# carlosmwh1985/BspAtom

Hardware: AMD Instinct MI355X
Metric: l-channel eigensolves/sec at N_bsp=4096 fp64 (higher is better)
Workload: dtype f64; 1 GPU; Hydrogen Coulomb l=0..127, N_bsp=4096, k=9, KIND_GRID=0 rb=800 (BASELINE configs[3]); `value` = weak scaling: 128 l-channels per GPU, 128 in total; channels_total=128, eigenvector_owner_rank=0, collective_calls=0, launched_by=python

## Files before the change

### bspatom_amd/csrc/capi.hip

```cpp
#include <atomic>
#include <new>
#include "capi_internal.h"

using namespace bsp;

namespace bsp {
static std::atomic<int> g_process_device{-1};
int process_device() { return g_process_device.load(); }
int process_device_check(int device)
{
    const int cur = g_process_device.load();
    if (cur >= 0 && cur != device) {
        fprintf(stderr, "bspatom: this process already works on device %d; use one process per GPU (device %d refused)\n", cur, device);
        return BSP_ERR_UNSUPPORTED;
    }
    return BSP_OK;
}
void process_device_latch(int device) { int expect = -1; g_process_device.compare_exchange_strong(expect, device); }
}

namespace {
struct OptName { const char *name; const char *env; int Options::*field; };
const OptName OPT_TABLE[] = {
    {"sb2st_version", "BSP_SB2ST_VERSION", &Options::sb2st_version},
    {"sb2st_ring", "BSP_SB2ST_RING", &Options::sb2st_ring},
    {"sb2st_margin", "BSP_SB2ST_MARGIN", &Options::sb2st_margin},
    {"sb2st_hyst", "BSP_SB2ST_HYST", &Options::sb2st_hyst},
    {"sb2st_lead", "BSP_SB2ST_LEAD", &Options::sb2st_lead},
    {"sb2st_check", "BSP_SB2ST_CHECK", &Options::sb2st_check},
    {"sb2st_diag", "BSP_SB2ST_DIAG", &Options::sb2st_diag},
    {"sb2st_force_abort", "BSP_SB2ST_FORCE_ABORT", &Options::sb2st_force_abort},
    {"sy2sb_groups", "BSP_SY2SB_GROUPS", &Options::sy2sb_groups},
    {"sy2sb_lookahead", "BSP_SY2SB_LOOKAHEAD", &Options::sy2sb_lookahead},
    {"sy2sb_segs", "BSP_SY2SB_SEGS", &Options::sy2sb_segs},
    {"panel_qr", "BSP_PANEL_QR", &Options::panel_qr},
    {"gemm_diag", "BSP_GEMM_DIAG", &Options::gemm_diag},
    {"bisect", "BSP_BISECT", &Options::bisect},
    {"bisect_ept", "BSP_BISECT_EPT", &Options::bisect_ept},
    {"bisect_tail", "BSP_BISECT_TAIL", &Options::bisect_tail},
    {"bisect_secant", "BSP_BISECT_SECANT", &Options::bisect_secant},
    {"bisect_pair", "BSP_BISECT_PAIR", &Options::bisect_pair},
    {"bisect_diag", "BSP_BISECT_DIAG", &Options::bisect_diag},
    {"no_eigvec_prefetch", "BSP_NO_EIGVEC_PREFETCH", &Options::no_eigvec_prefetch},
    {"vec_early", "BSP_VEC_EARLY", &Options::vec_early},
    {"vec_own_cu", "BSP_VEC_OWN_CU", &Options::vec_own_cu},
    {"poison_c", "BSP_POISON_C", &Options::poison_c},
    {"sb2sb_mfma", "BSP_SB2SB_MFMA", &Options::sb2sb_mfma},
    {"ktime", "BSP_KTIME", &Options::ktime},
    {"tsqr_regcap", "BSP_TSQR_REGCAP", &Options::tsqr_regcap},
    {"tsqr_max_m", "BSP_TSQR_MAX_M", &Options::tsqr_max_m},
    {"sb16_rows", "BSP_SB16_ROWS", &Options::sb16_rows},
    {"route", "BSP_ROUTE", &Options::route},
    {"cw_onediv", "BSP_CW_ONEDIV", &Options::cw_onediv},
    {"cw_items4", "BSP_CW_ITEMS4", &Options::cw_items4},
    {"cw_nw", "BSP_CW_NW", &Options::cw_nw},
    {"cw_ldspad", "BSP_CW_LDSPAD", &Options::cw_ldspad},
    {"cw_ipw", "BSP_CW_IPW", &Options::cw_ipw},
    {"cw_band8", "BSP_CW_BAND8", &Options::cw_band8},
    {"cw_split", "BSP_CW_SPLIT", &Options::cw_split},
    {"cw_diag", "BSP_CW_DIAG", &Options::cw_diag},
    {"s_overlap", "BSP_S_OVERLAP", &Options::s_overlap},
    {"cw_streams", "BSP_CW_STREAMS", &Options::cw_streams},
    {"cw_chunk_min", "BSP_CW_CHUNK_MIN", &Options::cw_chunk_min},
    {"sb8_wgs", "BSP_SB8_WGS", &Options::sb8_wgs},
    {"sbr_phased", "BSP_SBR_PHASED", &Options::sbr_phased},
    {"sbr_lag", "BSP_SBR_LAG", &Options::sbr_lag},
    {"fused_probe", "BSP_FUSED_PROBE", &Options::fused_probe},
    {"dipole_stage_mb", "BSP_DIPOLE_STAGE_MB", &Options::dipole_stage_mb},
    {"wf_stage_mb", "BSP_WF_STAGE_MB", &Options::wf_stage_mb},
    {"tdse_stage_mb", "BSP_TDSE_STAGE_MB", &Options::tdse_stage_mb},
};
}

namespace bsp {
Options &opts()
{
    static Options o = [] {
        Options v;
        for (const OptName &t : OPT_TABLE) {
            const char *e = getenv(t.env);
            if (e) v.*(t.field) = (*e == 0) ? 1 : atoi(e);
        }
        return v;
    }();
    return o;
}

namespace {
struct KRec { int slot; hipEvent_t e0, e1; };
std::vector<KRec> g_krecs;
std::vector<hipEvent_t> g_kpool;
hipEvent_t g_kopen[KS_COUNT];
hipEvent_t kevent()
{
    hipEvent_t e = nullptr;
    if (!g_kpool.empty()) { e = g_kpool.back(); g_kpool.pop_back(); }
    else if (hipEventCreate(&e) != hipSuccess) e = nullptr;
    return e;
}
const char *const KSLOT_NAMES[KS_COUNT] = {"gemm2_kernel<128,128,MODE 1> (rank-128 update, syr2k)", "gemm2_kernel<64,128,MODE 2> (symm Y = A22 W)",
                                          "panel_qr2_kernel / panel_qr_kernel", "sy2sb chain: G, K (split-K gemm_kernel + splitk_reduce), form_T, tsmm64 (W, Z)",
                                          "sb2sb_mfma_kernel (band 64 -> 16)", "sbr_rows_kernel<8> / <16> / sb16st_kernel (one-column chase to tridiagonal)", "bisect3_kernel",
                                          "band_cholesky_kernel + std_form_kernel",
                                          "crawford_item_kernel and its set-up kernels (band route: pencil -> band 15)",
                                          "operator_band_kernel (bands of caller-given g(r), g(r) d/dr)",
                                          "tdse_stage_kernel (one Runge-Kutta stage of bspatom_tdse_propagate)"};
}
void ktime_begin(int slot, hipStream_t st)
{
    hipEvent_t e = kevent();
    g_kopen[slot] = e;
    if (e) (void)hipEventRecord(e, st);
}
void ktime_end(int slot, hipStream_t st)
{
    hipEvent_t e0 = g_kopen[slot], e1 = kevent();
    g_kopen[slot] = nullptr;
    if (!e0 || !e1) return;
    (void)hipEventRecord(e1, st);
    g_krecs.push_back({slot, e0, e1});
}
}

extern "C" int bspatom_kernel_times(double *ms, int32_t *launches, int cap)
// ... 481 lines not shown
```

### bspatom_amd/csrc/common.h

```cpp
#pragma once
#include <hip/hip_runtime.h>
#include <cstdint>
#include <cstdio>
#include <cstdlib>

#define BSP_OK 0
#define BSP_ERR_HIP (-1)
#define BSP_ERR_ARG (-2)
#define BSP_ERR_BSPLVB (-3)
#define BSP_ERR_NOGPU (-4)
#define BSP_ERR_UNSUPPORTED (-5)

#define BSP_HIP(x)                                                                          \
    do {                                                                                    \
        hipError_t e_ = (x);                                                                \
        if (e_ != hipSuccess) {                                                             \
            fprintf(stderr, "bspatom: HIP error '%s' at %s:%d\n", hipGetErrorString(e_),    \
                    __FILE__, __LINE__);                                                    \
            return BSP_ERR_HIP;                                                             \
        }                                                                                   \
    } while (0)

typedef double double4_t __attribute__((ext_vector_type(4)));

__host__ __device__ inline size_t ab_stride(int npad) { return (size_t)npad * 128 + 1088; }

namespace bsp {

struct Options {
    int sb2st_version = 0;
    int sb2st_ring = 0;
    int sb2st_margin = 3, sb2st_hyst = 2;
    int sb2st_lead = 0;
    int sb2st_check = 0;
    int sb2st_diag = 0;
    int sb2st_force_abort = 0;
    int sy2sb_groups = 2, sy2sb_lookahead = 1, sy2sb_segs = 0;
    int panel_qr = 3;
    int tsqr_max_m = 2048;
    int tsqr_regcap = 1;
    int gemm_diag = 0;
    int bisect = 3, bisect_ept = 0;
    int bisect_secant = 1;
    int bisect_tail = 1;
    int bisect_pair = 1;
    int bisect_diag = 0;
    int no_eigvec_prefetch = 0;
    int vec_early = 1;
    int vec_own_cu = 1;
    int sb2sb_mfma = 1;
    int sb16_rows = 1;
    int poison_c = 0;
    int route = 0;
    int fused_probe = 0;
    int cw_items4 = 1;
    int cw_nw = 1;
    int cw_streams = 2;
    int cw_chunk_min = 1024;
    int s_overlap = 1;
    int cw_diag = 0;
    int cw_split = 0;
    int cw_band8 = 1;
    int sb8_wgs = 0;
    int sbr_phased = 1;
    int sbr_lag = 0;
    int cw_ipw = 0;
    int cw_ldspad = 0;
    int cw_onediv = 0;
    int dipole_stage_mb = 0;
    int wf_stage_mb = 0;
    int tdse_stage_mb = 0;
    int ktime = 0;
};
Options &opts();

int process_device();
int process_device_check(int device);
void process_device_latch(int device);

enum KSlot { KS_SYR2K = 0, KS_SYMM, KS_PANEL_QR, KS_CHAIN, KS_SB2SB, KS_SB16ST, KS_BISECT, KS_STDFORM, KS_CRAWFORD, KS_OPBAND, KS_TDSE, KS_COUNT };
void ktime_begin(int slot, hipStream_t st);
void ktime_end(int slot, hipStream_t st);
struct KScope {
    int slot; hipStream_t st; bool on;
    KScope(int slot_, hipStream_t st_) : slot(slot_), st(st_), on(opts().ktime != 0) { if (on) ktime_begin(slot, st); }
    ~KScope() { if (on) ktime_end(slot, st); }
};

struct GemmDesc {
    int M, N, K, batch;
    const double *A; long sAm, sAk, bA;
    const double *B; long sBk, sBn, bB;
    double *C; long sCm, sCn, bC;
    double alpha, beta;
    int lower_only;
    int yoff;
    int ksplit;
    int kchunk;
    long bCs;
    int nsb, toff;
    int sbpre[80];
    int sbxy[80];
};
int gemm_f64(const GemmDesc &g, hipStream_t st);
int gemm_splitk_f64(const GemmDesc &g, int splits, double *part, hipStream_t st);
int tsmm64_f64(int m, int batch, const double *A, long lda, long bsA, const double *B, long bsB, double *C, long ldc, long bsC,
               double alpha, double beta, hipStream_t st);
int syr2k_lower_f64(int m, int batch, double *A22, long ld, long bsA, const double *buf, long ldb, long bsBuf, int seg, int nseg,
                    int part, hipStream_t st);
int symm_lower_f64(int m, int batch, const double *A22, long ld, long bsA, const double *W, long ldw, long bsW,
                   double *Y, long ldy, long bsY, hipStream_t st);

int launch_point_table(int nkp, int k, int ka, int nfun, const double *d_rt, const double *d_aind,
                       const double *d_xg, const double *d_wg, const double *d_vpot, double *d_ptab,
                       int *d_left, int *d_status, hipStream_t st);
int launch_assemble_bands(int nfun, int k, int ka, int nkp, int kind_pot, const double *d_bl, int l0,
                          int nl, const double *d_ptab, const int *d_left, double *d_SB, double *d_HB,
                          hipStream_t st);
int launch_dipole_bands(int nfun, int k, int ka, int nkp, const double *d_ptab, const int *d_left, double *d_RB,
                        hipStream_t st);
int launch_band_cholesky(int n, int k, const double *d_SB, double *d_UB, double *d_rdiag, int *d_info,
                         hipStream_t st);
int launch_band_cholesky_range(int n, int k, int jstart, int jstop, const double *d_SB, double *d_UB, double *d_rdiag, int *d_info,
                               hipStream_t st);
int launch_band_cholesky_pair(int n, int k, int jstop, const double *d_SB, double *d_UB, double *d_rdiag, int *d_info, hipStream_t st);
int launch_standard_form(int n, int npad, int k, int nl, const double *d_HB, const double *d_UB,
                         const double *d_rdiag, double *d_Y, double *d_C, hipStream_t st, int full = 0);
struct CrawfordWork {
// ... 109 lines not shown
```

### bspatom_amd/csrc/tridiag.hip

```cpp
#include <vector>
#include "common.h"

namespace bsp {

__device__ __forceinline__ int sturm_count(const double *__restrict__ d, const double *__restrict__ e2,
                                           int n, double x, double pivmin)
{
    double q = d[0] - x;
    if (fabs(q) < pivmin) q = -pivmin;
    int cnt = (q < 0.0) ? 1 : 0;
    for (int i = 1; i < n; ++i) {
        q = (d[i] - x) - e2[i - 1] / q;
        if (fabs(q) < pivmin) q = -pivmin;
        cnt += (q < 0.0) ? 1 : 0;
    }
    return cnt;
}

constexpr int EPT = 4;

__global__ __launch_bounds__(256) void bisect_kernel(int n, int ldn, const double *__restrict__ dall,
                                                    const double *__restrict__ eall, double *wall, long ldw)
{
    extern __shared__ double sm[];
    double *d = sm, *e2 = sm + n;
    __shared__ double red[8];
    const int tid = threadIdx.x;
    const size_t ch = blockIdx.y;
    const double *dg = dall + ch * (size_t)ldn, *eg = eall + ch * (size_t)ldn;
    double gl = 1e300, gu = -1e300, emax = 0.0;
    for (int i = tid; i < n; i += 256) {
        const double di = dg[i];
        const double el = (i > 0) ? fabs(eg[i - 1]) : 0.0;
        const double er = (i < n - 1) ? fabs(eg[i]) : 0.0;
        d[i] = di;
        e2[i] = (i < n - 1) ? eg[i] * eg[i] : 0.0;
        gl = fmin(gl, di - el - er);
        gu = fmax(gu, di + el + er);
        emax = fmax(emax, er * er);
    }
#pragma unroll
    for (int off = 32; off >= 1; off >>= 1) {
        gl = fmin(gl, __shfl_xor(gl, off));
        gu = fmax(gu, __shfl_xor(gu, off));
        emax = fmax(emax, __shfl_xor(emax, off));
    }
    if ((tid & 63) == 0) { red[tid >> 6] = gl; red[4 + (tid >> 6)] = gu; }
    __syncthreads();
    gl = fmin(fmin(red[0], red[1]), fmin(red[2], red[3]));
    gu = fmax(fmax(red[4], red[5]), fmax(red[6], red[7]));
    __syncthreads();
    if ((tid & 63) == 0) red[tid >> 6] = emax;
    __syncthreads();
    emax = fmax(fmax(red[0], red[1]), fmax(red[2], red[3]));
    const double safmin = 2.2250738585072014e-308;
    const double pivmin = safmin * fmax(1.0, emax);
    const double tnorm = fmax(fabs(gl), fabs(gu));
    const double eps = 2.220446049250313e-16;
    gl = gl - 2.1 * tnorm * eps * n - 2.1 * pivmin;
    gu = gu + 2.1 * tnorm * eps * n + 2.1 * pivmin;

    const int mbase = blockIdx.x * (256 * EPT) + tid;
    double lo[EPT], hi[EPT];
#pragma unroll
    for (int c = 0; c < EPT; ++c) { lo[c] = gl; hi[c] = gu; }
    for (int it = 0; it < 128; ++it) {
        double mid[EPT];
        bool done[EPT];
        bool alld = true;
#pragma unroll
        for (int c = 0; c < EPT; ++c) {
            mid[c] = 0.5 * (lo[c] + hi[c]);
            done[c] = (mid[c] <= lo[c]) || (mid[c] >= hi[c]) ||
                      (hi[c] - lo[c] <= 2.0 * eps * fmax(fabs(lo[c]), fabs(hi[c])) + 2.0 * pivmin);
            alld = alld && done[c];
        }
        if (__syncthreads_and(alld)) break;
        double q[EPT];
        int cnt[EPT];
        {
            const double d0 = d[0];
#pragma unroll
// ... 137 lines not shown
            _Pragma("unroll") for (int r = 0; r < RS; ++r) {                                          \
                const double2 v = LOADROW(ib + sb * RS + r + 1);                                      \
                _Pragma("unroll") for (int c = 0; c < EPT; ++c) {                                     \
                    const double pn = __builtin_fma(v.x - x[c], p1[c], -(v.y * p0[c]));               \
                    h[c] = __builtin_amdgcn_alignbit(h[c], (unsigned)__double2hiint(pn), 31);         \
                    p0[c] = p1[c];                                                                    \
                    p1[c] = pn;                                                                       \
                }                                                                                     \
            }                                                                                         \
            _Pragma("unroll") for (int c = 0; c < EPT; ++c) {                                         \
                const int ex = -__builtin_amdgcn_frexp_exp(p1[c]);      \
                p1[c] = __builtin_amdgcn_ldexp(p1[c], ex);                                            \
                p0[c] = __builtin_amdgcn_ldexp(p0[c], ex);                                            \
                if (VAL) es[c] -= ex;                                            \
            }                                                                                         \
        }                                                                                             \
        _Pragma("unroll") for (int c = 0; c < EPT; ++c) {                                             \
            const unsigned t = __builtin_amdgcn_alignbit(hp[c], h[c], 1);                             \
            cnt[c] += __builtin_popcount(h[c] ^ t);                                                   \
            hp[c] = h[c];                                                                             \
        }                                                                                             \
    }
__device__ __forceinline__ double2 sturm_gload(const double2 *p)
{
    typedef double d2v __attribute__((ext_vector_type(2)));
    const d2v v = __builtin_nontemporal_load(reinterpret_cast<const d2v *>(p));
    return make_double2(v.x, v.y);
}
template <int EPT, bool VAL = false>
__device__ __forceinline__ void sturm_counts3(const double2 *__restrict__ de, int np, const double (&x)[EPT], int (&cnt)[EPT],
                                              const double2 *__restrict__ gt = nullptr, int nl = 0x7fffffff, float *lf = nullptr)
{
    double p0[EPT], p1[EPT];
    unsigned h[EPT], hp[EPT];
    int es[EPT];
#pragma unroll
    for (int c = 0; c < EPT; ++c) es[c] = 0;
    const double d0 = de[0].x;
#pragma unroll
    for (int c = 0; c < EPT; ++c) {
        p0[c] = 1.0; p1[c] = d0 - x[c];
        hp[c] = (unsigned)__double2hiint(p1[c]) >> 31;
        cnt[c] = (int)hp[c]; h[c] = 0u;
    }
    const int nlds = nl < np ? nl : np;
#define STURM_LDS(i) de[i]
#define STURM_GLB(i) sturm_gload(gt + (i))
    for (int ib = 0; ib < nlds; ib += HW) STURM_BLOCK(STURM_LDS)
    for (int ib = nlds; ib < np; ib += HW) STURM_BLOCK(STURM_GLB)
#undef STURM_LDS
#undef STURM_GLB
    if (VAL) {
#pragma unroll
        for (int c = 0; c < EPT; ++c) {
            const int e2 = __builtin_amdgcn_frexp_exp(p1[c]);
            const float mant = (float)__builtin_amdgcn_ldexp(p1[c], -e2);
            lf[c] = (float)(es[c] + e2) + __log2f(fmaxf(fabsf(mant), 1e-30f));
        }
    }
}

__device__ __forceinline__ double msect_point(double a, double w, int q, double rp)
{
    return __builtin_fma(w, (double)(q + 1) * rp, a);
}

__device__ __forceinline__ bool bracket_final(double lo, double hi)
{
    const double mid = 0.5 * (lo + hi);
    return (mid <= lo) || (mid >= hi) || (hi - lo <= 2.0 * 2.220446049250313e-16 * fmax(fabs(lo), fabs(hi)) + 1e-300);
}

__device__ __forceinline__ double uniform_double(double v)
{
    return __hiloint2double(__builtin_amdgcn_readfirstlane(__double2hiint(v)), __builtin_amdgcn_readfirstlane(__double2loint(v)));
}

static size_t bisect3_lds_bytes(int n, int ng)
{
    const int np = (n + HW - 1) / HW * HW;
    return (size_t)(np + 1) * 16 + (size_t)(ng / 2) * 16 + (size_t)ng * 4 + (size_t)(ng / 2) * 4;
}

constexpr int BISECT_DIAG_WORDS = 8;
template <int EPT, int TPB, bool DIAG = false>
__global__ __launch_bounds__(TPB) void bisect3_kernel(int n, int ldn, const double *__restrict__ dall,
                                                     const double *__restrict__ eall, double *wall, long ldw, int tail,
                                                     double2 *gtail, int nl, int hybrid_arg, int pair_stride, long long *diag)
{
    long long dt0 = DIAG ? (long long)wall_clock64() : 0;
    const int hybrid = EPT > 4 ? 0 : hybrid_arg;
    extern __shared__ double2 sde[];
    constexpr int NG = TPB * EPT;
    constexpr int NW = TPB / 64;
    constexpr int KC = NG / 2;
    const int np = (n + HW - 1) / HW * HW;
    const int nlr = nl < np ? nl : np;
    double2 *de = sde;
    const int kcap = hybrid ? NG / 4 : KC;
    double *llo = (double *)(sde + nlr + 1);
    double *lhi = llo + kcap;
    int *cg = (int *)(lhi + kcap);
    int *lm = cg + NG;
    __shared__ double red[2 * NW];
    __shared__ int sK;
    const int tid0 = threadIdx.x;
    const size_t ch = blockIdx.y;
    const double *dg = dall + ch * (size_t)ldn, *eg = eall + ch * (size_t)ldn;
    double *wout = wall + ch * (size_t)ldw;
    double2 *gt = gtail ? gtail + ch * (size_t)(np + 1) : nullptr;
    double gl = 1e300, gu = -1e300;
    for (int i = tid0; i < n; i += TPB) {
        const double di = dg[i];
        const double el = (i > 0) ? fabs(eg[i - 1]) : 0.0;
        const double er = (i < n - 1) ? fabs(eg[i]) : 0.0;
        gl = fmin(gl, di - el - er);
        gu = fmax(gu, di + el + er);
    }
#pragma unroll
    for (int off = 32; off >= 1; off >>= 1) {
        gl = fmin(gl, __shfl_xor(gl, off));
        gu = fmax(gu, __shfl_xor(gu, off));
    }
    if ((tid0 & 63) == 0) { red[tid0 >> 6] = gl; red[NW + (tid0 >> 6)] = gu; }
    __syncthreads();
#pragma unroll
    for (int q = 0; q < NW; ++q) { gl = fmin(gl, red[q]); gu = fmax(gu, red[NW + q]); }
    const double eps = 2.220446049250313e-16;
    double tnorm = fmax(fabs(gl), fabs(gu));
    if (!(tnorm > 0.0)) tnorm = 1.0;
    int kexp;
    (void)frexp(tnorm, &kexp);
    const double sc = ldexp(1.0, -kexp), isc_v = ldexp(1.0, kexp);
    for (int i = tid0; i <= np; i += TPB) {
        const double di = (i < n) ? dg[i] * sc : 2.0;
        const double ev = (i >= 1 && i < n) ? (eg[i - 1] * sc) : 0.0;
        const double2 row = make_double2(di, fmax(ev * ev, 1e-60));
        if (i <= nlr) de[i] = row; else gt[i] = row;
    }
    if (gt) asm volatile("s_waitcnt vmcnt(0)" ::: "memory");
    __syncthreads();
    gl = gl * sc - 2.1 * eps * n - 1e-300;
    gu = gu * sc + 2.1 * eps * n + 1e-300;

    gl = uniform_double(gl); gu = uniform_double(gu);
    const double isc = uniform_double(isc_v);
    const int nwl = (n + NG - 1) / NG;
#pragma unroll 1
    for (int item = 0; item < 2; ++item) {
        const int bx = blockIdx.x + item * pair_stride;
        if (item) {
            if (pair_stride == 0 || bx >= nwl) break;
            __syncthreads();
            if (DIAG) dt0 = (long long)wall_clock64();
        }
        int drounds = 0, dtail = 0;
        int tid = tid0;
        asm volatile("" : "+v"(tid));
        const int mbase = bx * NG + tid;
        double lo[EPT], hi[EPT];
        int clo[EPT], chi[EPT];
        float lflo[EPT], lfhi[EPT];
        if (!hybrid) {
            const double w = gu - gl;
            double xg[EPT];
            int cc[EPT];
#pragma unroll
            for (int c = 0; c < EPT; ++c) xg[c] = gl + w * ((double)(tid + TPB * c + 1) * (1.0 / (NG + 1)));
            if (DIAG) ++drounds;
            sturm_counts3<EPT>(de, np, xg, cc, gt, nlr);
#pragma unroll
            for (int c = 0; c < EPT; ++c) cg[tid + TPB * c] = cc[c];
            __syncthreads();
#pragma unroll
            for (int c = 0; c < EPT; ++c) {
                const int m = mbase + TPB * c;
                int L = -1, R = NG;
                while (R - L > 1) {
                    const int mid = (L + R) >> 1;
                    if (cg[mid] > m) R = mid; else L = mid;
                }
                lo[c] = (L < 0) ? gl : gl + w * ((double)(L + 1) * (1.0 / (NG + 1)));
                hi[c] = (R >= NG) ? gu : gl + w * ((double)(R + 1) * (1.0 / (NG + 1)));
                clo[c] = (L < 0) ? 0 : cg[L];
                chi[c] = (R >= NG) ? n : cg[R];
            }
        }
        bool done[EPT];
        if (hybrid) {
            double *xs = llo;
            float *lfs = (float *)(xs + NG);
            unsigned short *cs = (unsigned short *)(lfs + NG);
            const int m0 = bx * NG, m1 = min(m0 + NG, n);
            float wref[EPT];
            int st[EPT];
#pragma unroll
            for (int c = 0; c < EPT; ++c) {
                wref[c] = 3e38f; st[c] = 0;
                lo[c] = gl; hi[c] = gu; clo[c] = 0; chi[c] = n; lflo[c] = 3e38f; lfhi[c] = 3e38f;
            }
            for (int it = 0; it < 200; ++it) {
                double x[EPT];
                bool sec[EPT];
                int rng[EPT];
#pragma unroll
                for (int c = 0; c < EPT; ++c) {
                    const int m = mbase + TPB * c;
                    const double wd = hi[c] - lo[c];
                    done[c] = (m >= n) || bracket_final(lo[c], hi[c]);
                    if ((float)wd <= 0.5f * wref[c]) { wref[c] = (float)wd; st[c] &= 3; }
                    const bool slow = (st[c] >> 2) >= 3;
                    st[c] += 4;
                    x[c] = 0.5 * (lo[c] + hi[c]); sec[c] = false; rng[c] = 0;
                    const int a = max(clo[c], m0), b = min(chi[c], m1);
                    if (chi[c] - clo[c] == 1 && lflo[c] < 1e38f && lfhi[c] < 1e38f && !slow && !done[c]) {
                        const double tiny = 2.0 * 2.220446049250313e-16 * fmax(fabs(lo[c]), fabs(hi[c]));
                        const float dl = fminf(fmaxf(lflo[c] - lfhi[c], -60.0f), 60.0f);
                        const double r = (double)exp2f(dl);
                        const double xe = fmin(fmax(lo[c] + wd * (r / (1.0 + r)), lo[c] + tiny), hi[c] - tiny);
                        if (xe > lo[c] && xe < hi[c]) { x[c] = xe; sec[c] = true; }
                    } else if (b - a > 1 && m >= a && m < b && !slow && !done[c]) {
                        const double xq = msect_point(lo[c], wd, m - a, 1.0 / (double)(b - a + 1));
                        if (xq > lo[c] && xq < hi[c]) { x[c] = xq; rng[c] = (a - m0) | ((b - m0) << 16); }
                    }
                }
                int tot = 0;
#pragma unroll
                for (int c = 0; c < EPT; ++c) tot += __syncthreads_count(!done[c]);
                if (tot <= (tail ? NG / hybrid : 0)) break;
                int cnt[EPT];
                float lf[EPT];
                if (DIAG) ++drounds;
                sturm_counts3<EPT, true>(de, np, x, cnt, gt, nlr, lf);
#pragma unroll
                for (int c = 0; c < EPT; ++c) {
                    xs[tid + TPB * c] = x[c]; cs[tid + TPB * c] = (unsigned short)cnt[c]; lfs[tid + TPB * c] = lf[c];
                }
// ... 43 lines not shown
            for (int c = 0; c < EPT; ++c) {
                if (!done[c]) {
                    if (cnt[c] > mbase + TPB * c) hi[c] = mid[c]; else lo[c] = mid[c];
                }
            }
        }
        if (tid == 0) sK = 0;
        __syncthreads();
#pragma unroll
        for (int c = 0; c < EPT; ++c) {
            const int m = mbase + TPB * c;
            done[c] = (m >= n) || bracket_final(lo[c], hi[c]);
            if (!done[c]) {
                const int pos = atomicAdd(&sK, 1);
                if (pos < kcap) { llo[pos] = lo[c]; lhi[pos] = hi[c]; lm[pos] = m; }
                else wout[m] = 0.5 * (lo[c] + hi[c]) * isc;
            } else if (m < n) wout[m] = 0.5 * (lo[c] + hi[c]) * isc;
        }
        __syncthreads();
        for (int round = 0; round < 128; ++round) {
            const int K = min(sK, kcap);
            if (K == 0) break;
            const int P = NG / K;
            const double rp = 1.0 / (double)(P + 1);
            double x[EPT];
            int cc[EPT];
#pragma unroll
            for (int c = 0; c < EPT; ++c) {
                const int s = tid + TPB * c, e = s / P, q = s - e * P;
                x[c] = 2.0;
                if (e < K) { const double a = llo[e]; x[c] = msect_point(a, lhi[e] - a, q, rp); }
            }
            if (DIAG) ++dtail;
            sturm_counts3<EPT>(de, np, x, cc, gt, nlr);
#pragma unroll
            for (int c = 0; c < EPT; ++c) cg[tid + TPB * c] = cc[c];
            __syncthreads();
            double nlo[EPT / 2], nhi[EPT / 2];
            int nm[EPT / 2];
            bool keep[EPT / 2];
#pragma unroll
            for (int j = 0; j < EPT / 2; ++j) {
                const int e = tid + TPB * j;
                keep[j] = false;
                if (e < K) {
                    const double a = llo[e], b = lhi[e], w = b - a;
                    const int m = lm[e];
                    const int *ce = cg + e * P;
                    int L = -1, R = P;
                    while (R - L > 1) {
                        const int mid = (L + R) >> 1;
                        if (ce[mid] > m) R = mid; else L = mid;
                    }
                    nlo[j] = (L < 0) ? a : msect_point(a, w, L, rp);
                    nhi[j] = (R >= P) ? b : msect_point(a, w, R, rp);
                    nm[j] = m;
                    if (bracket_final(nlo[j], nhi[j]) || !(nhi[j] - nlo[j] < w)) wout[m] = 0.5 * (nlo[j] + nhi[j]) * isc;
                    else keep[j] = true;
                }
            }
            __syncthreads();
            if (tid == 0) sK = 0;
            __syncthreads();
#pragma unroll
            for (int j = 0; j < EPT / 2; ++j) {
                if (keep[j]) {
                    const int pos = atomicAdd(&sK, 1);
                    llo[pos] = nlo[j]; lhi[pos] = nhi[j]; lm[pos] = nm[j];
                }
            }
            __syncthreads();
        }
        {
            const int K = min(sK, kcap);
            for (int e = tid; e < K; e += TPB) wout[lm[e]] = 0.5 * (llo[e] + lhi[e]) * isc;
        }
        if (DIAG && tid == 0) {
            long long *rec = diag + (ch * (size_t)nwl + bx) * BISECT_DIAG_WORDS;
            rec[0] = bx; rec[1] = (long long)ch;
            rec[2] = (long long)(__builtin_amdgcn_s_getreg((31 << 11) | 20) & 0xfu);
            rec[3] = (long long)(unsigned)__builtin_amdgcn_s_getreg((31 << 11) | 4);
            rec[4] = dt0; rec[5] = (long long)wall_clock64();
            rec[6] = drounds; rec[7] = dtail;
        }
    }
}

__global__ __launch_bounds__(64) void bisect_one_kernel(int n, const double *__restrict__ dg, const double *__restrict__ eg,
                                                       int m, double *out)
{
    extern __shared__ double sm[];
    const int np = (n + RS - 1) / RS * RS;
    double *d = sm, *e2 = sm + np + RS;
    const int lane = threadIdx.x;
    double gl = 1e300, gu = -1e300;
    for (int i = lane; i < n; i += 64) {
        const double di = dg[i];
        const double el = (i > 0) ? fabs(eg[i - 1]) : 0.0;
        const double er = (i < n - 1) ? fabs(eg[i]) : 0.0;
        gl = fmin(gl, di - el - er);
        gu = fmax(gu, di + el + er);
    }
#pragma unroll
    for (int off = 32; off >= 1; off >>= 1) {
        gl = fmin(gl, __shfl_xor(gl, off));
        gu = fmax(gu, __shfl_xor(gu, off));
    }
    const double eps = 2.220446049250313e-16;
    double tnorm = fmax(fabs(gl), fabs(gu));
    if (!(tnorm > 0.0)) tnorm = 1.0;
    int kexp;
    (void)frexp(tnorm, &kexp);
    const double sc = ldexp(1.0, -kexp), isc = ldexp(1.0, kexp);
    for (int i = lane; i < np + RS; i += 64) {
        d[i] = (i < n) ? dg[i] * sc : 2.0;
        const double ev = (i < n - 1) ? (eg[i] * sc) : 0.0;
        e2[i] = fmax(ev * ev, 1e-60);
    }
    __syncthreads();
    double lo = gl * sc - 2.1 * eps * n - 1e-300, hi = gu * sc + 2.1 * eps * n + 1e-300;
    for (int round = 0; round < 40; ++round) {
        if (hi - lo <= 2.0 * eps * fmax(fabs(lo), fabs(hi)) + 1e-300) break;
        const double w = (hi - lo) * (1.0 / 65.0);
        const double x = lo + (lane + 1) * w;
        if (!(x > lo && x < hi)) {
            const double mid = 0.5 * (lo + hi);
            if (!(mid > lo && mid < hi)) break;
        }
        double p0 = 1.0, p1 = d[0] - x;
        int cnt = (p1 < 0.0) ? 1 : 0;
        for (int ib = 0; ib < np; ib += RS) {
#pragma unroll
            for (int r = 0; r < RS; ++r) {
                const int i = ib + r + 1;
                const double pn = __builtin_fma(d[i] - x, p1, -(e2[i - 1] * p0));
                cnt += (int)((unsigned)(__double2hiint(pn) ^ __double2hiint(p1)) >> 31);
                p0 = p1; p1 = pn;
            }
            int ea, eb;
            (void)frexp(p1, &ea);
            (void)frexp(p0, &eb);
            const int ex = (p1 == 0.0) ? eb : ((p0 == 0.0) ? ea : max(ea, eb));
            p1 = ldexp(p1, -ex); p0 = ldexp(p0, -ex);
        }
        const unsigned long long above = __ballot(cnt > m);
        const int f = above ? (__ffsll((long long)above) - 1) : 64;
        const double xl = __shfl(x, f > 0 ? f - 1 : 0), xh = __shfl(x, f < 64 ? f : 63);
        const double nlo = (f > 0) ? xl : lo, nhi = (f < 64) ? xh : hi;
        if (!(nhi - nlo < hi - lo)) break;
        lo = nlo; hi = nhi;
    }
    if (lane == 0) *out = 0.5 * (lo + hi) * isc;
}

__global__ __launch_bounds__(256) void bisect_one3_kernel(int n, const double *__restrict__ dg, const double *__restrict__ eg,
                                                         int m, double *out)
{
    extern __shared__ double2 sde[];
    constexpr int NG = 256 * EPT;
    const int np = (n + HW - 1) / HW * HW;
    double2 *de = sde;
    int *cg = (int *)(sde + np + 1);
    __shared__ double red[8];
    const int tid = threadIdx.x;
    double gl = 1e300, gu = -1e300;
    for (int i = tid; i < n; i += 256) {
// ... 48 lines not shown
        lo = nlo; hi = nhi;
    }
    if (tid == 0) *out = 0.5 * (lo + hi) * isc;
}

int launch_bisect_one(int n, const double *d_d, const double *d_e, int m, double *d_out, hipStream_t st)
{
    const int variant1 = opts().bisect;
    if (variant1 >= 3) {
        const size_t lds3 = (size_t)2 * (n + 3 * RS + HW) * sizeof(double) + 256 * EPT * sizeof(int);
        if (lds3 > 150 * 1024) return BSP_ERR_UNSUPPORTED;
        static bool attr3 = false;
        if (!attr3) {
            BSP_HIP(hipFuncSetAttribute(reinterpret_cast<const void *>(bisect_one3_kernel),
                                        hipFuncAttributeMaxDynamicSharedMemorySize, 150 * 1024));
            attr3 = true;
        }
        hipLaunchKernelGGL(bisect_one3_kernel, dim3(1), dim3(256), lds3, st, n, d_d, d_e, m, d_out);
        BSP_HIP(hipGetLastError());
        return BSP_OK;
    }
    const size_t lds = (size_t)2 * (n + 3 * RS) * sizeof(double);
    if (lds > 150 * 1024) return BSP_ERR_UNSUPPORTED;
    static bool attr = false;
    if (!attr) {
        BSP_HIP(hipFuncSetAttribute(reinterpret_cast<const void *>(bisect_one_kernel),
                                    hipFuncAttributeMaxDynamicSharedMemorySize, 150 * 1024));
        attr = true;
    }
    hipLaunchKernelGGL(bisect_one_kernel, dim3(1), dim3(64), lds, st, n, d_d, d_e, m, d_out);
    BSP_HIP(hipGetLastError());
    return BSP_OK;
}

int launch_bisect(int n, int ldn, int batch, const double *d_d, const double *d_e, double *d_w, long ldw,
                  hipStream_t st)
{
    const int ept_env = opts().bisect_ept;
    int mode = (ept_env == 8) ? 8 : (ept_env == 4) ? 4 : (ept_env == 2) ? 1024 : (ept_env == 21) ? 21 : (ept_env == 5) ? 512 : 22;
    int ng = (mode == 4) ? 1024 : (mode == 21 ? 512 : (mode == 22 ? 1024 : 2048));
    if (bisect3_lds_bytes(n, ng) > 150 * 1024) { mode = 22; ng = 1024; }
    const int np3 = (n + HW - 1) / HW * HW;
    int nl = np3;
    while (bisect3_lds_bytes(nl, ng) > 150 * 1024) nl -= HW;
    const size_t lds3 = bisect3_lds_bytes(nl, ng);
    const size_t lds = (size_t)2 * (n + 3 * RS + HW) * sizeof(double);
    struct Tail { hipStream_t st; double2 *p; size_t cap; };
    static std::vector<Tail> g_tails;
    double2 *gtail = nullptr;
    if (nl < np3) {
        const size_t need = (size_t)batch * (np3 + 1);
        Tail *tl = nullptr;
        for (auto &x : g_tails) if (x.st == st) tl = &x;
        if (!tl) { g_tails.push_back({st, nullptr, 0}); tl = &g_tails.back(); }
        if (need > tl->cap) {
            if (tl->p) { BSP_HIP(hipStreamSynchronize(st)); (void)hipFree(tl->p); tl->p = nullptr; tl->cap = 0; }
            BSP_HIP(hipMalloc(reinterpret_cast<void **>(&tl->p), need * sizeof(double2)));
            tl->cap = need;
        }
        gtail = tl->p;
        if (opts().bisect < 3) return BSP_ERR_UNSUPPORTED;
    }
    static bool attr_set = false;
    const int variant = opts().bisect;
    if (!attr_set) {
        BSP_HIP(hipFuncSetAttribute(reinterpret_cast<const void *>(bisect_kernel),
                                    hipFuncAttributeMaxDynamicSharedMemorySize, 150 * 1024));
        BSP_HIP(hipFuncSetAttribute(reinterpret_cast<const void *>(bisect2_kernel),
                                    hipFuncAttributeMaxDynamicSharedMemorySize, 150 * 1024));
        BSP_HIP(hipFuncSetAttribute(reinterpret_cast<const void *>(bisect3_kernel<4, 256>),
                                    hipFuncAttributeMaxDynamicSharedMemorySize, 150 * 1024));
        BSP_HIP(hipFuncSetAttribute(reinterpret_cast<const void *>(bisect3_kernel<8, 256>),
                                    hipFuncAttributeMaxDynamicSharedMemorySize, 150 * 1024));
        BSP_HIP(hipFuncSetAttribute(reinterpret_cast<const void *>(bisect3_kernel<4, 512>),
                                    hipFuncAttributeMaxDynamicSharedMemorySize, 150 * 1024));
        BSP_HIP(hipFuncSetAttribute(reinterpret_cast<const void *>(bisect3_kernel<2, 1024>),
                                    hipFuncAttributeMaxDynamicSharedMemorySize, 150 * 1024));
        BSP_HIP(hipFuncSetAttribute(reinterpret_cast<const void *>(bisect3_kernel<2, 256>),
                                    hipFuncAttributeMaxDynamicSharedMemorySize, 150 * 1024));
        BSP_HIP(hipFuncSetAttribute(reinterpret_cast<const void *>(bisect3_kernel<2, 512>),
                                    hipFuncAttributeMaxDynamicSharedMemorySize, 150 * 1024));
        BSP_HIP(hipFuncSetAttribute(reinterpret_cast<const void *>(bisect3_kernel<2, 512, true>),
                                    hipFuncAttributeMaxDynamicSharedMemorySize, 150 * 1024));
        attr_set = true;
    }
    const dim3 grid((n + 256 * EPT - 1) / (256 * EPT), batch);
    if (variant == 1 || variant == 2) {
        KScope kt(KS_BISECT, st);
        if (variant == 1) hipLaunchKernelGGL(bisect_kernel, grid, dim3(256), lds, st, n, ldn, d_d, d_e, d_w, ldw);
        else hipLaunchKernelGGL(bisect2_kernel, grid, dim3(256), lds, st, n, ldn, d_d, d_e, d_w, ldw);
        BSP_HIP(hipGetLastError());
        return BSP_OK;
    }
    static int cus = 0;
    if (!cus) {
        int dev = 0;
        BSP_HIP(hipGetDevice(&dev));
        BSP_HIP(hipDeviceGetAttribute(&cus, hipDeviceAttributeMultiprocessorCount, dev));
    }
    const int nw = (n + ng - 1) / ng;
    const int pmode = opts().bisect_pair;
    const int pair_stride = (pmode == 2 || (pmode == 1 && (long)nw * batch > cus)) ? (nw + 1) / 2 : 0;
    const dim3 g3(pair_stride ? pair_stride : nw, batch);
    const int tail = opts().bisect_tail;
    const int hyb = n > 65535 ? 0 : (opts().bisect_secant == 1 ? 8 : (opts().bisect_secant >= 4 ? opts().bisect_secant : (opts().bisect_secant >= 2 ? 4 : 0)));
#define BISECT3_LAUNCH(E, T, D, dbuf) hipLaunchKernelGGL((bisect3_kernel<E, T, D>), g3, dim3(T), lds3, st, n, ldn, d_d, d_e, d_w, ldw, tail, gtail, nl, hyb, \
                                                         pair_stride, dbuf)
    if (opts().bisect_diag) {
        if (mode != 22) {
            fprintf(stderr, "bspatom: BSP_BISECT_DIAG is built for the default workgroup shape only (512 x 2)\n");
            return BSP_ERR_UNSUPPORTED;
        }
        const size_t words = (size_t)nw * batch * BISECT_DIAG_WORDS;
        std::vector<long long> h(words);
        long long *dbuf = nullptr;
        BSP_HIP(hipMalloc(reinterpret_cast<void **>(&dbuf), words * sizeof(long long)));
        BSP_HIP(hipMemsetAsync(dbuf, 0, words * sizeof(long long), st));
        BISECT3_LAUNCH(2, 512, true, dbuf);
        const hipError_t le = hipGetLastError();
        if (le != hipSuccess) { hipFree(dbuf); BSP_HIP(le); }
        BSP_HIP(hipStreamSynchronize(st));
        BSP_HIP(hipMemcpy(h.data(), dbuf, words * sizeof(long long), hipMemcpyDeviceToHost));
        hipFree(dbuf);
        int dev = 0, khz = 0;
        BSP_HIP(hipGetDevice(&dev));
        BSP_HIP(hipDeviceGetAttribute(&khz, hipDeviceAttributeWallClockRate, dev));
        fprintf(stderr, "bisect3 diag: n %d batch %d nw %d pair_stride %d grid %u x %u lds %zu cus %d wall_khz %d\n", n, batch, nw, pair_stride,
                g3.x, g3.y, lds3, cus, khz);
        for (size_t r = 0; r < (size_t)nw * batch; ++r) {
            const long long *q = h.data() + r * BISECT_DIAG_WORDS;
            fprintf(stderr, "bisect3 wg: x %lld ch %lld xcc %lld hwid 0x%llx t0 %lld t1 %lld rounds %lld tail %lld\n", q[0], q[1], q[2], q[3], q[4], q[5],
                    q[6], q[7]);
        }
        return BSP_OK;
    }
    KScope kt(KS_BISECT, st);
    if (mode == 512) BISECT3_LAUNCH(4, 512, false, nullptr);
    else if (mode == 1024) BISECT3_LAUNCH(2, 1024, false, nullptr);
    else if (mode == 8) BISECT3_LAUNCH(8, 256, false, nullptr);
    else if (mode == 21) BISECT3_LAUNCH(2, 256, false, nullptr);
    else if (mode == 22) BISECT3_LAUNCH(2, 512, false, nullptr);
    else BISECT3_LAUNCH(4, 256, false, nullptr);
#undef BISECT3_LAUNCH
    BSP_HIP(hipGetLastError());
    return BSP_OK;
}

}
```

Before: 2010 eigensolves/s.

## Add atomic work-queue scheduling for bisection eigenvalue kernel

```diff
diff --git a/bspatom_amd/csrc/capi.hip b/bspatom_amd/csrc/capi.hip
--- a/bspatom_amd/csrc/capi.hip
+++ b/bspatom_amd/csrc/capi.hip
@@ -40,6 +40,8 @@
     {"bisect_tail", "BSP_BISECT_TAIL", &Options::bisect_tail},
     {"bisect_secant", "BSP_BISECT_SECANT", &Options::bisect_secant},
     {"bisect_pair", "BSP_BISECT_PAIR", &Options::bisect_pair},
+    {"bisect_queue", "BSP_BISECT_QUEUE", &Options::bisect_queue},
+    {"bisect_queue_grid", "BSP_BISECT_QUEUE_GRID", &Options::bisect_queue_grid},
     {"bisect_diag", "BSP_BISECT_DIAG", &Options::bisect_diag},
     {"no_eigvec_prefetch", "BSP_NO_EIGVEC_PREFETCH", &Options::no_eigvec_prefetch},
     {"vec_early", "BSP_VEC_EARLY", &Options::vec_early},
diff --git a/bspatom_amd/csrc/common.h b/bspatom_amd/csrc/common.h
--- a/bspatom_amd/csrc/common.h
+++ b/bspatom_amd/csrc/common.h
@@ -44,6 +44,8 @@
     int bisect_secant = 1;
     int bisect_tail = 1;
     int bisect_pair = 1;
+    int bisect_queue = 1;
+    int bisect_queue_grid = 0;
     int bisect_diag = 0;
     int no_eigvec_prefetch = 0;
     int vec_early = 1;
diff --git a/bspatom_amd/csrc/tridiag.hip b/bspatom_amd/csrc/tridiag.hip
--- a/bspatom_amd/csrc/tridiag.hip
+++ b/bspatom_amd/csrc/tridiag.hip
@@ -1,3 +1,4 @@
+#include <algorithm>
 #include <vector>
 #include "common.h"
 
@@ -301,11 +302,14 @@
     return (size_t)(np + 1) * 16 + (size_t)(ng / 2) * 16 + (size_t)ng * 4 + (size_t)(ng / 2) * 4;
 }
 
-constexpr int BISECT_DIAG_WORDS = 8;
-template <int EPT, int TPB, bool DIAG = false>
+constexpr int BISECT_DIAG_WORDS = 10;
+constexpr int BISECT_Q_CUS = 16 * 256;
+constexpr int BISECT_Q_WORDS = BISECT_Q_CUS + 4;
+template <int EPT, int TPB, bool DIAG = false, bool QUEUE = false>
 __global__ __launch_bounds__(TPB) void bisect3_kernel(int n, int ldn, const double *__restrict__ dall,
                                                      const double *__restrict__ eall, double *wall, long ldw, int tail,
-                                                     double2 *gtail, int nl, int hybrid_arg, int pair_stride, long long *diag)
+                                                     double2 *gtail, int nl, int hybrid_arg, int pair_stride, long long *diag,
+                                                     unsigned *qcnt, int items, int batch)
 {
     long long dt0 = DIAG ? (long long)wall_clock64() : 0;
     const int hybrid = EPT > 4 ? 0 : hybrid_arg;
@@ -323,55 +327,89 @@
     int *lm = cg + NG;
     __shared__ double red[2 * NW];
     __shared__ int sK;
+    __shared__ int sItem, sSide;
     const int tid0 = threadIdx.x;
-    const size_t ch = blockIdx.y;
-    const double *dg = dall + ch * (size_t)ldn, *eg = eall + ch * (size_t)ldn;
-    double *wout = wall + ch * (size_t)ldw;
-    double2 *gt = gtail ? gtail + ch * (size_t)(np + 1) : nullptr;
-    double gl = 1e300, gu = -1e300;
-    for (int i = tid0; i < n; i += TPB) {
-        const double di = dg[i];
-        const double el = (i > 0) ? fabs(eg[i - 1]) : 0.0;
-        const double er = (i < n - 1) ? fabs(eg[i]) : 0.0;
-        gl = fmin(gl, di - el - er);
-        gu = fmax(gu, di + el + er);
-    }
-#pragma unroll
-    for (int off = 32; off >= 1; off >>= 1) {
-        gl = fmin(gl, __shfl_xor(gl, off));
-        gu = fmax(gu, __shfl_xor(gu, off));
-    }
-    if ((tid0 & 63) == 0) { red[tid0 >> 6] = gl; red[NW + (tid0 >> 6)] = gu; }
-    __syncthreads();
-#pragma unroll
-    for (int q = 0; q < NW; ++q) { gl = fmin(gl, red[q]); gu = fmax(gu, red[NW + q]); }
-    const double eps = 2.220446049250313e-16;
-    double tnorm = fmax(fabs(gl), fabs(gu));
-    if (!(tnorm > 0.0)) tnorm = 1.0;
-    int kexp;
-    (void)frexp(tnorm, &kexp);
-    const double sc = ldexp(1.0, -kexp), isc_v = ldexp(1.0, kexp);
-    for (int i = tid0; i <= np; i += TPB) {
-        const double di = (i < n) ? dg[i] * sc : 2.0;
-        const double ev = (i >= 1 && i < n) ? (eg[i - 1] * sc) : 0.0;
-        const double2 row = make_double2(di, fmax(ev * ev, 1e-60));
-        if (i <= nlr) de[i] = row; else gt[i] = row;
-    }
-    if (gt) asm volatile("s_waitcnt vmcnt(0)" ::: "memory");
-    __syncthreads();
-    gl = gl * sc - 2.1 * eps * n - 1e-300;
-    gu = gu * sc + 2.1 * eps * n + 1e-300;
-
-    gl = uniform_double(gl); gu = uniform_double(gu);
-    const double isc = uniform_double(isc_v);
+    size_t ch = blockIdx.y;
+    double *wout;
+    double2 *gt;
+    double gl, gu, isc;
+    const auto channel_setup = [&]() __attribute__((always_inline)) {
+        const double *dg = dall + ch * (size_t)ldn, *eg = eall + ch * (size_t)ldn;
+        wout = wall + ch * (size_t)ldw;
+        gt = gtail ? gtail + ch * (size_t)(np + 1) : nullptr;
+        gl = 1e300; gu = -1e300;
+        for (int i = tid0; i < n; i += TPB) {
+            const double di = dg[i];
+            const double el = (i > 0) ? fabs(eg[i - 1]) : 0.0;
+            const double er = (i < n - 1) ? fabs(eg[i]) : 0.0;
+            gl = fmin(gl, di - el - er);
+            gu = fmax(gu, di + el + er);
+        }
+#pragma unroll
+        for (int off = 32; off >= 1; off >>= 1) {
+            gl = fmin(gl, __shfl_xor(gl, off));
+            gu = fmax(gu, __shfl_xor(gu, off));
+        }
+        if ((tid0 & 63) == 0) { red[tid0 >> 6] = gl; red[NW + (tid0 >> 6)] = gu; }
+        __syncthreads();
+#pragma unroll
+        for (int q = 0; q < NW; ++q) { gl = fmin(gl, red[q]); gu = fmax(gu, red[NW + q]); }
+        const double eps = 2.220446049250313e-16;
+        double tnorm = fmax(fabs(gl), fabs(gu));
+        if (!(tnorm > 0.0)) tnorm = 1.0;
+        int kexp;
+        (void)frexp(tnorm, &kexp);
+        const double sc = ldexp(1.0, -kexp), isc_v = ldexp(1.0, kexp);
+        for (int i = tid0; i <= np; i += TPB) {
+            const double di = (i < n) ? dg[i] * sc : 2.0;
+            const double ev = (i >= 1 && i < n) ? (eg[i - 1] * sc) : 0.0;
+            const double2 row = make_double2(di, fmax(ev * ev, 1e-60));
+            if (i <= nlr) de[i] = row; else gt[i] = row;
+        }
+        if (gt) asm volatile("s_waitcnt vmcnt(0)" ::: "memory");
+        __syncthreads();
+        gl = gl * sc - 2.1 * eps * n - 1e-300;
+        gu = gu * sc + 2.1 * eps * n + 1e-300;
+
+        gl = uniform_double(gl); gu = uniform_double(gu);
+        isc = uniform_double(isc_v);
+    };
     const int nwl = (n + NG - 1) / NG;
+    int side = -1;
+    if (QUEUE) {
+        if (tid0 == 0) {
+            const unsigned xcc = __builtin_amdgcn_s_getreg((31 << 11) | 20) & 0xfu;
+            const unsigned cu = (__builtin_amdgcn_s_getreg((31 << 11) | 4) >> 8) & 0xffu;
+            sSide = (int)atomicAdd(qcnt + xcc * 256 + cu, 1u);
+        }
+    } else
+        channel_setup();
 #pragma unroll 1
-    for (int item = 0; item < 2; ++item) {
-        const int bx = blockIdx.x + item * pair_stride;
-        if (item) {
-            if (pair_stride == 0 || bx >= nwl) break;
+    for (int item = 0; QUEUE || item < 2; ++item) {
+        int bx;
+        if (QUEUE) {
+            if (item) __syncthreads();
+            if (tid0 == 0) {
+                int it = -1;
+                if (atomicAdd(qcnt + BISECT_Q_CUS, 1u) < (unsigned)items)
+                    it = (sSide & 1) ? items - 1 - (int)atomicAdd(qcnt + BISECT_Q_CUS + 2, 1u) : (int)atomicAdd(qcnt + BISECT_Q_CUS + 1, 1u);
+                sItem = it;
+            }
             __syncthreads();
-            if (DIAG) dt0 = (long long)wall_clock64();
+            const int it = __builtin_amdgcn_readfirstlane(sItem);
+            if (it < 0) break;
+            if (DIAG) { dt0 = (long long)wall_clock64(); side = __builtin_amdgcn_readfirstlane(sSide); }
+            const int rank = it / batch;
+            bx = (rank & 1) ? (rank >> 1) : nwl - 1 - (rank >> 1);
+            const size_t chn = (size_t)(it - rank * batch);
+            if (item == 0 || chn != ch) { ch = chn; channel_setup(); }
+        } else {
+            bx = blockIdx.x + item * pair_stride;
+            if (item) {
+                if (pair_stride == 0 || bx >= nwl) break;
+                __syncthreads();
+                if (DIAG) dt0 = (long long)wall_clock64();
+            }
         }
         int drounds = 0, dtail = 0;
         int tid = tid0;
@@ -581,6 +619,7 @@
             rec[3] = (long long)(unsigned)__builtin_amdgcn_s_getreg((31 << 11) | 4);
             rec[4] = dt0; rec[5] = (long long)wall_clock64();
             rec[6] = drounds; rec[7] = dtail;
+            rec[8] = (long long)(blockIdx.x + gridDim.x * blockIdx.y); rec[9] = side;
         }
     }
 }
@@ -795,6 +834,10 @@
                                     hipFuncAttributeMaxDynamicSharedMemorySize, 150 * 1024));
         BSP_HIP(hipFuncSetAttribute(reinterpret_cast<const void *>(bisect3_kernel<2, 512, true>),
                                     hipFuncAttributeMaxDynamicSharedMemorySize, 150 * 1024));
+        BSP_HIP(hipFuncSetAttribute(reinterpret_cast<const void *>(bisect3_kernel<2, 512, false, true>),
+                                    hipFuncAttributeMaxDynamicSharedMemorySize, 150 * 1024));
+        BSP_HIP(hipFuncSetAttribute(reinterpret_cast<const void *>(bisect3_kernel<2, 512, true, true>),
+                                    hipFuncAttributeMaxDynamicSharedMemorySize, 150 * 1024));
         attr_set = true;
     }
     const dim3 grid((n + 256 * EPT - 1) / (256 * EPT), batch);
@@ -813,12 +856,29 @@
     }
     const int nw = (n + ng - 1) / ng;
     const int pmode = opts().bisect_pair;
-    const int pair_stride = (pmode == 2 || (pmode == 1 && (long)nw * batch > cus)) ? (nw + 1) / 2 : 0;
-    const dim3 g3(pair_stride ? pair_stride : nw, batch);
+    const int qmode = opts().bisect_queue;
+    const long items = (long)nw * batch;
+    const bool queue = mode == 22 && items < (1L << 30) && (qmode == 2 || (qmode == 1 && items > cus));
+    const int pair_stride = queue ? 0 : ((pmode == 2 || (pmode == 1 && items > cus)) ? (nw + 1) / 2 : 0);
+    int qgrid = (int)std::min(items, 2L * cus);
+    if (opts().bisect_queue_grid > 0) qgrid = std::min(qgrid, opts().bisect_queue_grid);
+    const dim3 g3 = queue ? dim3(qgrid, 1) : dim3(pair_stride ? pair_stride : nw, batch);
+    struct QCount { hipStream_t st; unsigned *p; };
+    static std::vector<QCount> g_qcounts;
+    unsigned *qcnt = nullptr;
+    if (queue) {
+        for (auto &x : g_qcounts) if (x.st == st) qcnt = x.p;
+        if (!qcnt) {
+            BSP_HIP(hipMalloc(reinterpret_cast<void **>(&qcnt), BISECT_Q_WORDS * sizeof(unsigned)));
+            g_qcounts.push_back({st, qcnt});
+        }
+        BSP_HIP(hipMemsetAsync(qcnt, 0, BISECT_Q_WORDS * sizeof(unsigned), st));
+    }
     const int tail = opts().bisect_tail;
     const int hyb = n > 65535 ? 0 : (opts().bisect_secant == 1 ? 8 : (opts().bisect_secant >= 4 ? opts().bisect_secant : (opts().bisect_secant >= 2 ? 4 : 0)));
-#define BISECT3_LAUNCH(E, T, D, dbuf) hipLaunchKernelGGL((bisect3_kernel<E, T, D>), g3, dim3(T), lds3, st, n, ldn, d_d, d_e, d_w, ldw, tail, gtail, nl, hyb, \
-                                                         pair_stride, dbuf)
+#define BISECT3_LAUNCH_Q(E, T, D, Q, dbuf) hipLaunchKernelGGL((bisect3_kernel<E, T, D, Q>), g3, dim3(T), lds3, st, n, ldn, d_d, d_e, d_w, ldw, tail, gtail, nl, \
+                                                              hyb, pair_stride, dbuf, qcnt, (int)items, batch)
+#define BISECT3_LAUNCH(E, T, D, dbuf) BISECT3_LAUNCH_Q(E, T, D, false, dbuf)
     if (opts().bisect_diag) {
         if (mode != 22) {
             fprintf(stderr, "bspatom: BSP_BISECT_DIAG is built for the default workgroup shape only (512 x 2)\n");
@@ -829,7 +889,8 @@
         long long *dbuf = nullptr;
         BSP_HIP(hipMalloc(reinterpret_cast<void **>(&dbuf), words * sizeof(long long)));
         BSP_HIP(hipMemsetAsync(dbuf, 0, words * sizeof(long long), st));
-        BISECT3_LAUNCH(2, 512, true, dbuf);
+        if (queue) BISECT3_LAUNCH_Q(2, 512, true, true, dbuf);
+        else BISECT3_LAUNCH(2, 512, true, dbuf);
         const hipError_t le = hipGetLastError();
         if (le != hipSuccess) { hipFree(dbuf); BSP_HIP(le); }
         BSP_HIP(hipStreamSynchronize(st));
@@ -838,12 +899,12 @@
         int dev = 0, khz = 0;
         BSP_HIP(hipGetDevice(&dev));
         BSP_HIP(hipDeviceGetAttribute(&khz, hipDeviceAttributeWallClockRate, dev));
-        fprintf(stderr, "bisect3 diag: n %d batch %d nw %d pair_stride %d grid %u x %u lds %zu cus %d wall_khz %d\n", n, batch, nw, pair_stride,
-                g3.x, g3.y, lds3, cus, khz);
+        fprintf(stderr, "bisect3 diag: n %d batch %d nw %d pair_stride %d queue %d grid %u x %u lds %zu cus %d wall_khz %d\n", n, batch, nw, pair_stride,
+                queue ? 1 : 0, g3.x, g3.y, lds3, cus, khz);
         for (size_t r = 0; r < (size_t)nw * batch; ++r) {
             const long long *q = h.data() + r * BISECT_DIAG_WORDS;
-            fprintf(stderr, "bisect3 wg: x %lld ch %lld xcc %lld hwid 0x%llx t0 %lld t1 %lld rounds %lld tail %lld\n", q[0], q[1], q[2], q[3], q[4], q[5],
-                    q[6], q[7]);
+            fprintf(stderr, "bisect3 wg: x %lld ch %lld xcc %lld hwid 0x%llx t0 %lld t1 %lld rounds %lld tail %lld hwg %lld side %lld\n", q[0], q[1], q[2], q[3],
+                    q[4], q[5], q[6], q[7], q[8], q[9]);
         }
         return BSP_OK;
     }
@@ -852,9 +913,11 @@
     else if (mode == 1024) BISECT3_LAUNCH(2, 1024, false, nullptr);
     else if (mode == 8) BISECT3_LAUNCH(8, 256, false, nullptr);
     else if (mode == 21) BISECT3_LAUNCH(2, 256, false, nullptr);
+    else if (mode == 22 && queue) BISECT3_LAUNCH_Q(2, 512, false, true, nullptr);
     else if (mode == 22) BISECT3_LAUNCH(2, 512, false, nullptr);
     else BISECT3_LAUNCH(4, 256, false, nullptr);
 #undef BISECT3_LAUNCH
+#undef BISECT3_LAUNCH_Q
     BSP_HIP(hipGetLastError());
     return BSP_OK;
 }
```

New measurement: 2042 eigensolves/s (median of 6 runs). 1.6% higher.
